# JoshElkind/concurrent-raytracer-go

Measured on AMD Instinct MI355X. Metric: Mrays/sec at 800x600x100spp max_depth=50 (sphere_reflections_light), higher is better.
Workload: dtype f64; 1 GPU; sphere_reflections_light_facing 800x600 100spp depth 50, soft shadows, recursive reflections; width=800, height=600, spp=100, max_depth=50, parallelism=1 GPU, frames_in_flight=64, frames_per_launch=32

## Files before the change

concurrent-raytracer-go_amd/csrc/rt_api.cpp:

```cpp
#include <math.h>
#include <stdlib.h>

#include <chrono>
#include <mutex>
#include <thread>

#include "rt_context.h"

namespace rtgo {

static thread_local std::string g_last_error;
void set_error(const std::string& msg) { g_last_error = msg; }

static int validate_scene(const rt_scene* s) {
  if (!s) {
    set_error("scene is NULL");
    return RT_E_INVALID;
  }
  if (s->num_objects < 0 || s->num_lights < 0 || (s->num_objects > 0 && !s->objects) ||
      (s->num_lights > 0 && !s->lights)) {
    set_error("scene arrays inconsistent");
    return RT_E_INVALID;
  }
  for (int i = 0; i < s->num_objects; ++i) {
// ... 221 lines not shown
  if (n > 0 && (!out || capacity < n)) {
    set_error("cone rows: out holds " + std::to_string(out ? capacity : 0) + " rows, the scene has " + std::to_string(n));
    return RT_E_INVALID;
  }
  FlatScene f;
  flatten_scene(*scene, &f);
  if ((force_bvh > 0 || (force_bvh == 0 && (f.spheres.size() > 64 || f.boxes.size() > (size_t)kAutoBvhCubes))) &&
      spheres_finite(f))
    build_bvh(&f, 0, 0);
  std::vector<unsigned long long> rows;
  cone_rows(f, &rows);
  for (size_t i = 0; i < n; ++i) out[i] = rows[i];
  return RT_OK;
}

int rt_stream_decode(int32_t order, uint32_t frames, uint32_t nlive, uint32_t spp, const uint32_t* entries, size_t n,
                     uint32_t* out) {
  if ((order != 0 && order != 1) || frames == 0 || nlive == 0 || spp == 0 || (n > 0 && (!entries || !out))) {
    set_error("stream decode: order is 0 or 1, frames, nlive and spp are at least 1, entries and out hold n");
    return RT_E_INVALID;
  }
  bool small = ((frames | nlive | spp) >> 31) == 0;
  for (size_t j = 0; j < n && small; ++j) small = (entries[j] >> 31) == 0;
  if (!small) {
    set_error("stream decode: frames, nlive, spp and every entry are below 2^31");
    return RT_E_INVALID;
  }
  const StreamDecode k = stream_decode_of(order, frames, nlive, spp);
  for (size_t j = 0; j < n; ++j) {
    const StreamEntry en = stream_decode(k, order, entries[j]);
    out[3 * j] = en.fl;
    out[3 * j + 1] = en.i;
    out[3 * j + 2] = en.s;
  }
  return RT_OK;
}

const char* rt_last_error(void) { return g_last_error.c_str(); }

constexpr size_t kStageDefault = 256 * 1024;
constexpr size_t kSmallDefault = 64 * 1024;

int rt_context_create(int32_t device, rt_context** out) {
  if (!out) {
    set_error("out is NULL");
    return RT_E_INVALID;
  }
  *out = nullptr;
  int n = 0;
  HIP_TRY(hipGetDeviceCount(&n));
  if (device < 0 || device >= n) {
    set_error("device " + std::to_string(device) + " out of range (" + std::to_string(n) + " devices)");
    return RT_E_DEVICE;
  }
  HIP_TRY(hipSetDevice(device));
  {
    static std::mutex mu;
    static std::vector<bool> loaded;
    std::lock_guard<std::mutex> lock(mu);
    if ((int)loaded.size() < n) loaded.resize(n, false);
    if (!loaded[device]) {
      hipError_t e = (hipError_t)preload_render_kernels();
      if (e == hipSuccess) e = (hipError_t)preload_sched_kernels();
      if (e == hipSuccess) e = (hipError_t)preload_wf_kernels();
      if (e != hipSuccess) {
        set_error(std::string("kernel code object load failed: ") + hipGetErrorString(e));
// ... 273 lines not shown
```

concurrent-raytracer-go_amd/csrc/rt_device.h:

```cpp
#pragma once
#include <hip/hip_runtime.h>

#include "../../include/rt_rng.h"
#include "rt_internal.h"

#ifdef RT_CHECK_XLANE
namespace rtgo {
__device__ unsigned long long g_xlane_faults;
}
template <typename T>
__device__ __forceinline__ T rt_checked_shfl(T v, int src, int width = 64) {
  const unsigned long long ex = __builtin_amdgcn_read_exec();
  const int lane = (int)(threadIdx.x & 63);
  const int from = (lane & ~(width - 1)) + (src & (width - 1));
  if (!((ex >> (from & 63)) & 1ull)) atomicAdd(&rtgo::g_xlane_faults, 1ull);
  return __shfl(v, src, width);
}
#define __shfl(...) rt_checked_shfl(__VA_ARGS__)
#endif

namespace rtgo {

struct d3 {
  double x, y, z;
// ... 112 lines not shown
__device__ __forceinline__ bool unit_ball_accept(uint32_t ux, uint32_t uy, uint32_t uz) {
  const float fx = __builtin_fmaf((float)ux, 0x1p-31f, -1.f), fy = __builtin_fmaf((float)uy, 0x1p-31f, -1.f),
              fz = __builtin_fmaf((float)uz, 0x1p-31f, -1.f);
  const float l = __builtin_fmaf(fz, fz, __builtin_fmaf(fy, fy, fx * fx));
  if (l < 1.f - 0x1p-16f) return true;
  if (l > 1.f + 0x1p-16f) return false;
  return len2(unit_ball_point(ux, uy, uz)) < 1;
}

template <bool kCount>
__device__ __forceinline__ d3 rand_in_unit_sphere(rt_rng& r, Counters& c) {
  for (;;) {
    const uint32_t ux = rt_rng_next(&r), uy = rt_rng_next(&r), uz = rt_rng_next(&r);
    cnt<kCount>(c, C_RNG, 3);
    if (unit_ball_accept(ux, uy, uz)) return unit_ball_point(ux, uy, uz);
  }
}

__device__ __forceinline__ double approx_rcp(double a) {
  const double r0 = __builtin_amdgcn_rcp(a);
  const double e = __builtin_fma(-a, r0, 1.0);
  return __builtin_fma(r0, e, r0);
}

__device__ __forceinline__ bool root_out(double num, double a, double inv_a, double tmin, double tmax) {
  const double r = num * inv_a;
  const double e = fabs(r) * 0x1p-40;
  if (r + e < tmin || r - e > tmax) return true;
  if (r - e >= tmin && r + e <= tmax) return false;
  const double q = num / a;
  return q < tmin || tmax < q;
}

__device__ __forceinline__ int sphere_query(const DSphere& S, d3 o, d3 d, double a, double inv_a, double tmin,
                                            double tmax, double& num) {
  double ocx = o.x - S.c[0], ocy = o.y - S.c[1], ocz = o.z - S.c[2];
  double hb = ocx * d.x + ocy * d.y + ocz * d.z;
  double c = (ocx * ocx + ocy * ocy + ocz * ocz) - S.r2;
  double disc = hb * hb - a * c;
  if (disc < 0) return 0;
  double sq = sqrt(disc);
  double n1 = -hb - sq;
  if (!root_out(n1, a, inv_a, tmin, tmax)) {
    num = n1;
    return 1;
  }
  double n2 = -hb + sq;
  if (!root_out(n2, a, inv_a, tmin, tmax)) {
    num = n2;
    return 2;
  }
  return 0;
}

__device__ __forceinline__ bool tri_test(const DTri& T, d3 o, d3 d, double tmin, double tmax, double& t,
                                         double& uo, double& vo) {
  d3 e1 = ld3(T.e1), e2 = ld3(T.e2);
  d3 h = cross(d, e2);
  double a = dot(e1, h);
  if (a > -1e-6 && a < 1e-6) return false;
  double f = 1.0 / a;
  d3 s = o - ld3(T.v0);
  double u = f * dot(s, h);
  if (u < 0.0 || u > 1.0) return false;
  d3 q = cross(s, e1);
  double v = f * dot(d, q);
  if (v < 0.0 || u + v > 1.0) return false;
  double tv = f * dot(e2, q);
  if (tv < tmin || tv > tmax) return false;
  t = tv;
  uo = u;
  vo = v;
  return true;
// ... 551 lines not shown
```

concurrent-raytracer-go_amd/csrc/rt_internal.h:

```cpp
#pragma once
#include <stdint.h>

#include <string>
#include <vector>

#include <hip/hip_runtime_api.h>

#include "../../include/rt_api.h"
#include "rt_scene_dev.h"

namespace rtgo {

void set_error(const std::string& msg);

int dev_alloc(void** p, size_t n);
void dev_free(void* p);
int host_alloc(void** p, size_t n, bool* fresh = nullptr);
void host_free(void* p);
int dev_stream_get(hipStream_t* s);
void dev_stream_put(hipStream_t s);
int dev_event_get(hipEvent_t* e);
void dev_event_put(hipEvent_t e);

struct FlatScene {
// ... 181 lines not shown
#define RT_HOST_DEVICE __host__ __device__
#else
#define RT_HOST_DEVICE
#endif
struct StreamDiv {
  uint32_t d, m, l, _pad;
};
struct StreamDecode {
  StreamDiv d0, d1;
};
struct StreamEntry {
  uint32_t fl, i, s;
};
inline StreamDiv stream_div_of(uint32_t d) {
  StreamDiv r{d, 0, 0, 0};
  while ((1ull << r.l) < d) ++r.l;
  r.m = (uint32_t)(((1ull << (31 + r.l)) + d - 1) / d);
  return r;
}
inline StreamDecode stream_decode_of(int32_t order, uint32_t frames, uint32_t nlive, uint32_t spp) {
  const uint32_t a = order == 0 ? spp : frames, b = order == 0 ? nlive : spp;
  return StreamDecode{stream_div_of(a ? a : 1u), stream_div_of(b ? b : 1u)};
}
template <class Div>
RT_HOST_DEVICE inline uint32_t stream_div(uint32_t n, const Div& k) {
  return (uint32_t)(((uint64_t)(n << 1) * k.m) >> 32) >> k.l;
}
template <class Decode>
RT_HOST_DEVICE inline StreamEntry stream_decode(const Decode& k, int32_t order, uint32_t e) {
  const uint32_t t = stream_div(e, k.d0), r0 = e - t * k.d0.d;
  const uint32_t q = stream_div(t, k.d1), r1 = t - q * k.d1.d;
  return order == 0 ? StreamEntry{q, r1, r0} : StreamEntry{r0, q, r1};
}
struct StreamParams {
  const int32_t* live;
  const int32_t* live_pos;
  const int32_t* tile_list;
  double* rows;
  unsigned int* cursor;
  uint32_t total;
  int32_t nlive, npix;
  int32_t frame0, frames;
  int32_t chunk, order;
  double* acc;
  const CamFrame* cams;
  StreamDecode dec;
};
struct StreamKArgs {
  KParams k;
  StreamParams s;
};
int launch_stream(const KParams& p, const StreamParams& sp, int wgs, void* stream);
constexpr int kStreamKernels = 6;
int stream_kernel_of(const KParams& p, bool cams = false);
struct CamTable {
  CamFrame f[kMaxFrames];
};
int launch_cam_upload(const CamTable& t, int n, CamFrame* d_cams, void* stream);
int stream_wave_slots(int device, int kernel, size_t shmem);

int launch_render(const KParams& p, bool count, void* stream);
size_t render_shmem(const KParams& p);
int launch_download(const void* d_src, void* h_dst_mapped, size_t bytes, void* stream);
int launch_spin(double ms, void* stream);
int partition_balanced(rt_context* c, int32_t w, int32_t h, const rt_settings* st, int32_t world, int measure_spp,
                       rt_partition** out);
// ... 146 lines not shown
```

concurrent-raytracer-go_amd/csrc/rt_kernel.hip:

```cpp
#include <hip/hip_runtime.h>

#include "../../include/rt_rng.h"
#include "rt_device.h"
#include "rt_internal.h"

#ifndef RT_WAVES_PER_SIMD
#define RT_WAVES_PER_SIMD 3
#endif
#ifndef RT_STREAM_SPH_WAVES
#define RT_STREAM_SPH_WAVES 4
#endif
#ifndef RT_COOP_MAX
#define RT_COOP_MAX 8
#endif
constexpr int kCoopMax = RT_COOP_MAX;
#ifndef RT_SQ_TAIL
#define RT_SQ_TAIL 2
#endif
constexpr int kSqTail = RT_SQ_TAIL;
#ifndef RT_SQ_TRIES
#define RT_SQ_TRIES 2
#endif
constexpr int kSqTries = RT_SQ_TRIES;
#ifndef RT_SOLO
// ... 63 lines not shown
      for (int j = 0; j < p.nb; ++j) {
        const DBox& B = p.boxes[j];
        const unsigned long long g = 0xFFFull << B.first;
        if ((m.t & g) && !ray_box(B, o, id, 0.001, tmax)) m.t &= ~g;
      }
    }
  }
  if (m.s) {
    const double a = len2(d);
    const double inv_a = approx_rcp(a);
    for (unsigned long long b = m.s; b; b &= b - 1) {
      const int i = __builtin_ctzll(b);
      cnt<kCount>(c, C_SPH);
      double num;
      if (sphere_query(p.spheres[i], o, d, a, inv_a, 0.001, tmax, num)) return true;
    }
  }
  if constexpr (!kSph) {
    for (unsigned long long b = m.t; b; b &= b - 1) {
      const int i = __builtin_ctzll(b);
      cnt<kCount>(c, C_TRI);
      double t, u, v;
      if (tri_test(p.tris[i], o, d, 0.001, tmax, t, u, v)) return true;
    }
  }
  return false;
}

template <bool kCount, bool kSph = false, bool kMix = false>
__device__ __forceinline__ bool shadow_blocked(const Geo& p, bool masks, d3 o, d3 d, double tmax,
                                               typename Kind<kSph>::C m, int* stack, Counters& c) {
  if (masks) return cand_any(m) && any_hit_masked<kCount, kSph>(p, o, d, tmax, m, c);
  return any_hit<kCount, kSph, kMix>(p, o, d, tmax, stack, c);
}

__device__ __forceinline__ int wide_groups(bool need, unsigned long long qmask, int nq, int* owner_tab, int& ow,
                                           int& k, bool& helper) {
  const int lane = (int)(threadIdx.x & 63);
  const int S = nq <= 4 ? 16 : (nq <= 8 ? 8 : 4);
  if (need) owner_tab[lanes_below(qmask)] = lane;
  __syncthreads();
  const int grp = lane / S;
  k = lane - grp * S;
  helper = grp < nq;
  ow = helper ? owner_tab[grp] : lane;
  __syncthreads();
  return S;
}

template <bool kCount, bool kSph = false>
__device__ __forceinline__ bool closest_wide(const Geo& g, bool need, unsigned long long qmask, int nq, d3 o, d3 d,
                                             typename Kind<kSph>::H& hs, bool& fallback, Counters& c) {
  __shared__ int owner_tab[16];
  const int lane = (int)(threadIdx.x & 63);
  int ow, k;
  bool helper;
  const int S = wide_groups(need, qmask, nq, owner_tab, ow, k, helper);
  const d3 ro = mk(__shfl(o.x, ow), __shfl(o.y, ow), __shfl(o.z, ow));
  const d3 rd = mk(__shfl(d.x, ow), __shfl(d.y, ow), __shfl(d.z, ow));
  const double a = len2(rd);
  const double inv_a = approx_rcp(a);
  double bt = __builtin_inf(), bnum = 0;
  int bobj = -1, bidx = -1;
  bool found = false;
  if (helper) {
    for (int i = k; i < g.ns; i += S) {
// ... 51 lines not shown
  unsigned long long m = 0;
  if (helper) {
    for (int i = k; i < g.ns; i += S) {
      const DSphere& Sp = g.spheres[i];
      if constexpr (kRows) {
        if (!((rowo >> i) & 1)) continue;
      }
      if (self_out && Sp.obj == selfo && Sp.r > 0) continue;
      if (in_cone(Sp.c, Sp.r, Po, Lo, dist)) m |= 1ull << i;
    }
  }
  for (int off = S >> 1; off >= 1; off >>= 1) m |= __shfl_xor(m, off);
  const int lead = need ? lanes_below(qmask) * S : lane;
  return __shfl(m, lead);
}

__device__ __forceinline__ bool light_inert(const DMat* m, const DLight& Lt, d3 N, d3 ldir, d3 D) {
  return gmax0(dot(N, ldir)) == 0.0 && D.x != 0.0 && D.y != 0.0 && D.z != 0.0 && __builtin_isfinite(Lt.intensity) &&
         __builtin_isfinite(Lt.color[0] + Lt.color[1] + Lt.color[2]) &&
         __builtin_isfinite(m->albedo[0] + m->albedo[1] + m->albedo[2]) && __builtin_isfinite(m->metallic) &&
         __builtin_isfinite(m->diffuse_strength);
}

struct CoopOut {
  uint64_t x;
  int unocc;
  int tries;
};
__device__ __forceinline__ Cand cand_of_lane(Cand m, int ow) { return Cand{rl64(m.s, ow), rl64(m.t, ow)}; }
__device__ __forceinline__ CandS cand_of_lane(CandS m, int ow) { return CandS{rl64(m.s, ow)}; }
template <bool kCount, bool kSph = false, bool kMix = false>
__device__ __forceinline__ CoopOut soft_coop(const Geo p, bool masks, bool trace, d3 P, d3 ldir, double ldist,
                             typename Kind<kSph>::C cm, uint64_t x, const uint64_t* jump, int* stack, Counters& c) {
  const int lane = (int)(threadIdx.x & 63);
  int need = 16, unocc = 0, tries = 0;
  while (need > 0) {
    const uint64_t x0 = state_at3(x, jump, lane), x1 = x0 * RT_PCG_MULT + RT_PCG_INC,
                   x2 = x1 * RT_PCG_MULT + RT_PCG_INC;
    const uint32_t o0 = rt_pcg_out(x0), o1 = rt_pcg_out(x1), o2 = rt_pcg_out(x2);
    const bool acc = unit_ball_accept(o0, o1, o2);
    const unsigned long long am = __ballot(acc);
    const int rank = lanes_below(am);
    const bool chosen = acc && rank < need;
    const unsigned long long chm = __ballot(chosen);
    const int nch = __popcll(chm);
    const int used = nch == need ? 64 - __clzll(chm) : 64;
    bool occ = false;
    if (chosen && trace)
      occ = shadow_blocked<kCount, kSph, kMix>(p, masks, P, normalize(ldir + muls(unit_ball_point(o0, o1, o2), 0.1)), ldist,
                                         cm, stack, c);
    unocc += nch - __popcll(__ballot(chosen && occ));
    need -= nch;
    tries += used;
    x = state_at3(x, jump, used);
  }
  return CoopOut{x, unocc, tries};
}

template <bool kCount, bool kSph = false, bool kMix = false>
__device__ __forceinline__ int soft_queue(const Geo& p, bool masks, bool need_soft, bool trace, d3 P, d3 ldir,
                                          double ldist, typename Kind<kSph>::C cm, rt_rng& rng, const uint64_t* jump,
                                          int* stack, Counters& c) {
  constexpr int kRingNeed = 64 * kSqTries + 64 + 16 * kSqTail;
  constexpr unsigned kRing = kRingNeed <= 256 ? 256u : (unsigned)kRingNeed;
  __shared__ uint4 sq[kRing];
  __shared__ int sq_unocc[64];
  const int lane = lane_now() & 63;
  sq_unocc[lane] = 0;
  int need = need_soft ? 16 : 0, free_rays = 0;
  int head = 0, tail = 0;
  for (;;) {
    constexpr int K = kSqTries;
    bool acc[K];
    uint32_t u[K][3];
#pragma unroll
    for (int t = 0; t < K; ++t) {
      acc[t] = false;
      u[t][0] = u[t][1] = u[t][2] = 0;
    }
    if (need > 0) {
      rt_rng r = rng;
#pragma unroll
      for (int t = 0; t < K; ++t) {
// ... 38 lines not shown
            const int nch = __popcll(chm);
            const int used = nch == nd ? 64 - __clzll(chm) : 64;
            if (tr) {
              if (chosen) sq[(unsigned)(tail + lanes_below(chm)) % kRing] = make_uint4(o0, o1, o2, (uint32_t)ow);
              tail += nch;
            }
            got += nch;
            nd -= nch;
            tries += used;
            x = state_at3(x, jump, used);
          }
          if (lane == ow) {
            rng.x = x;
            need = 0;
            if (!tr) free_rays += got;
            cnt<kCount>(c, C_RNG, 3ull * tries);
            cnt<kCount>(c, C_SHADOW, got);
          }
        }
      }
    }
    const bool more = __ballot(need > 0) != 0;
    while (tail - head >= 64 || (!more && tail > head)) {
      __syncthreads();
      const int n = min(64, tail - head);
      const uint4 e = sq[(unsigned)(head + lane) % kRing];
      const int ow = lane < n ? (int)e.w : lane;
      const d3 Po = mk(__shfl(P.x, ow), __shfl(P.y, ow), __shfl(P.z, ow));
      const d3 Lo = mk(__shfl(ldir.x, ow), __shfl(ldir.y, ow), __shfl(ldir.z, ow));
      const double dist = __shfl(ldist, ow);
      typename Kind<kSph>::C co;
      co.s = __shfl(cm.s, ow);
      if constexpr (!kSph) co.t = p.nt ? __shfl(cm.t, ow) : 0ull;
      if (lane < n) {
        const d3 pt = mk(rt_bits_to_unit(e.x) * 2 - 1, rt_bits_to_unit(e.y) * 2 - 1, rt_bits_to_unit(e.z) * 2 - 1);
        if (!shadow_blocked<kCount, kSph, kMix>(p, masks, Po, normalize(Lo + muls(pt, 0.1)), dist, co, stack, c))
          atomicAdd(&sq_unocc[ow], 1);
      }
      head += n;
      __syncthreads();
    }
    if (!more && head == tail) break;
  }
  __syncthreads();
  return need_soft ? sq_unocc[lane] + free_rays : 0;
}


typedef const __attribute__((address_space(4))) KParams* KArg;
__device__ __forceinline__ KArg fresh() {
  KArg k = (KArg)__builtin_amdgcn_kernarg_segment_ptr();
  asm volatile("" : "+s"(k));
  return k;
}

__device__ __forceinline__ unsigned main_wg(KArg k) {
  const unsigned b = blockIdx.x;
  return (k->tail != nullptr && b >= (unsigned)k->tail_pos) ? b - (unsigned)k->tail_helpers : b;
}
__device__ __forceinline__ int frame_of(KArg k) {
  return k->nframes > 1 ? (int)(main_wg(k) % (unsigned)k->nframes) : 0;
}
__device__ __forceinline__ int block_of(KArg k) {
  return k->nframes > 1 ? (int)(main_wg(k) / (unsigned)k->nframes) : (int)main_wg(k);
}
__device__ __forceinline__ size_t split_index(KArg k, int slot) {
  return (size_t)frame_of(k) * (size_t)k->nsplit + (size_t)slot;
}

struct BlockLoc {
  int lt, tile, tx, ty;
// ... 84 lines not shown
    const bool mine = ((row >> i) & 1) != 0 && !(sphere_out && S.obj == self && S.r > 0);
    if (__ballot(mine) == 0) continue;
    if (mine && in_cone(S.c, S.r, P, ldir, ldist)) m.s |= 1ull << i;
  }
  return m;
}

__device__ __forceinline__ CamK cam_k(KArg k) {
  return make_cam(k->frame_key[frame_of(k)], k->W, k->H, k->cf);
}
template <bool kCount>
__device__ __forceinline__ void camera_ray(KArg k, int x, int y, int s, rt_rng& rng, d3& o, d3& d, Counters& c) {
  camera_ray_c<kCount>(cam_k(k), k->cf, x, y, s, rng, o, d, c);
}

enum WgSection { kClkHit, kClkLight, kClkSoft, kClkHard, kClkScat };
#ifdef RT_WG_TIMING
__shared__ unsigned long long solo_clk[16];
struct WgClock {
  unsigned long long t_start = 0, t_loop = 0, iter = 0;
  unsigned long long sec[5] = {0, 0, 0, 0, 0}, from[5] = {0, 0, 0, 0, 0};
  unsigned long long vis = 0, alive = 0, coop = 0, seq = 0;
  unsigned long long rf_top = 0, rf_top_lanes = 0, rf_second = 0, rf_second_lanes = 0;
  typedef unsigned long long Buckets __attribute__((ext_vector_type(5)));
  Buckets bclk = {0, 0, 0, 0, 0}, bcnt = {0, 0, 0, 0, 0};
  unsigned long long bts = 0;
  int bprev = -1;
  unsigned long long solo_t0 = 0;
  unsigned long long first = 0, last = 0, last_d0 = 0, last_d1 = 0, paths = 0, solo = 0, bounces = 0;

  __device__ __forceinline__ unsigned long long* record(KArg k) const { return k->dbg + (size_t)blockIdx.x * kDbgStride; }
  __device__ __forceinline__ void start(int lane) {
    if (lane < 16) solo_clk[lane] = 0;
    t_start = __builtin_amdgcn_s_memrealtime();
    vis = __builtin_amdgcn_s_memtime();
  }
  __device__ __forceinline__ void visibility_done() { vis = __builtin_amdgcn_s_memtime() - vis; }
  __device__ __forceinline__ void iteration(bool is_alive, int lane) {
    ++iter;
    alive += __popcll(__ballot(is_alive));
    {
      const unsigned long long now = __builtin_amdgcn_s_memtime();
      if (bprev >= 0) bclk[bprev] += now - bts;
      const int nal = __popcll(__ballot(is_alive));
      bprev = nal == 1 ? 0 : (nal == 2 ? 1 : (nal <= 4 ? 2 : (nal <= 8 ? 3 : 4)));
      bcnt[bprev] += 1;
      bts = now;
    }
    if (iter % 4 == 0 && iter / 4 < 16 && lane == 0 && fresh()->dbg) record(fresh())[16 + iter / 4] = __builtin_amdgcn_s_memrealtime();
    from[kClkHit] = __builtin_amdgcn_s_memtime();
  }
  __device__ __forceinline__ void begin(WgSection s) { from[s] = __builtin_amdgcn_s_memtime(); }
  __device__ __forceinline__ void end(WgSection s) { sec[s] += __builtin_amdgcn_s_memtime() - from[s]; }
  __device__ __forceinline__ void hit_done() {
    from[kClkLight] = __builtin_amdgcn_s_memtime();
    sec[kClkHit] += from[kClkLight] - from[kClkHit];
  }
  __device__ __forceinline__ void soft_form(unsigned long long owners) {
    if (__popcll(owners) <= kCoopMax) coop += __popcll(owners); else ++seq;
  }
  __device__ __forceinline__ void refill(bool second, unsigned long long served) {
    if (served == 0) return;
    if (second) {
      rf_second += 1;
      rf_second_lanes += __popcll(served);
    } else {
      rf_top += 1;
      rf_top_lanes += __popcll(served);
    }
  }
  __device__ __forceinline__ void loop_done() {
    t_loop = __builtin_amdgcn_s_memrealtime();
    if (bprev >= 0) bclk[bprev] += __builtin_amdgcn_s_memtime() - bts;
  }
  __device__ __forceinline__ void write(KArg k, int lane, bool block, unsigned long long shape, unsigned long long split) const {
    if (k->dbg && lane == 0) {
      unsigned long long* r = record(k);
      r[0] = t_start;
      r[1] = t_loop;
      r[2] = __builtin_amdgcn_s_memrealtime();
      r[3] = sec[kClkHit];
      r[4] = sec[kClkLight];
      r[5] = sec[kClkSoft];
      r[6] = vis;
      r[7] = iter;
      r[8] = sec[kClkHard];
      r[9] = sec[kClkScat];
      r[10] = alive;
      r[11] = coop;
      r[12] = seq;
      r[13] = shape;
      r[14] = split;
      for (int i = 0; i < 5; ++i) {
        r[32 + i] = bclk[i];
        r[37 + i] = bcnt[i];
      }
      if (block && solo_clk[6])
        for (int i = 0; i < 16; ++i) r[16 + i] = solo_clk[i];
      r[42] = block ? solo_clk[6] : 0;
      r[43] = block ? solo_clk[7] : 0;
      r[44] = rf_top;
      r[45] = rf_top_lanes;
      r[46] = rf_second;
      r[47] = rf_second_lanes;
    }
  }
  __device__ __forceinline__ void stream_write(int lane) const { write(fresh(), lane, false, 0, 0); }
  __device__ __forceinline__ void solo_start() { solo_t0 = __builtin_amdgcn_s_memtime(); }
  __device__ __forceinline__ void solo_count(int k) { solo_clk[k] += 1; }
  __device__ __forceinline__ void solo_lap(int k) {
    const unsigned long long now = __builtin_amdgcn_s_memtime();
    solo_clk[k] += now - solo_t0;
    solo_t0 = now;
  }
  __device__ __forceinline__ void solo_mark(int k) { solo_clk[k] += __builtin_amdgcn_s_memtime() - solo_t0; }
  __device__ __forceinline__ void helper_path(unsigned long long t_path, int d0, int d1) {
    if (!first) first = t_path;
    paths += 1;
    solo += __builtin_amdgcn_s_memrealtime() - t_path;
    last = t_path;
    last_d0 = (unsigned long long)d0;
    last_d1 = (unsigned long long)d1;
    bounces += (unsigned long long)(d1 - d0);
  }
  __device__ __forceinline__ void helper_write(KArg k, int lane, unsigned long long t_born) const {
// ... 1951 lines not shown
```

concurrent-raytracer-go_amd/rtgo/__init__.py:

```python
from __future__ import annotations

import ctypes
import json
import os
import time
from datetime import datetime, timezone

import numpy as np

_HERE = os.path.dirname(os.path.abspath(__file__))
LIB_PATH = os.environ.get("RTGO_LIB") or os.path.join(os.path.dirname(_HERE), "build", "librtgo.so")

RT_OK = 0
RT_E_TIMEOUT = -6
RT_OBJ_SPHERE, RT_OBJ_CUBE = 0, 1
MATERIAL_KINDS = {
    "lambertian": 0,
    "metal": 1,
    "shiny": 2,
    "perfectmirror": 3,
    "glass": 4,
    "dielectric": 5,
    "diffuselight": 6,
}
# ... 235 lines not shown
    "rt_partition_tile",
    "rt_partition_max_local",
    "rt_partition_packed_bytes",
    "rt_partition_rgba_offset",
    "rt_partition_work",
    "rt_context_set_partition",
    "rt_unpack_partition_async",
    "rt_comm_gather_bytes_async",
    "rt_renderer_rank_seconds",
    "rt_renderer_num_ranks",
    "rt_debug_xlane_faults",
    "rt_context_tail_debug",
    "rt_context_profile",
    "rt_context_kernel_seconds",
    "rt_context_render_frames_async",
    "rt_unpack_partition_frames_async",
    "rt_release_cached_memory",
    "rt_renderer_set_watchdog",
    "rt_renderer_test_stall",
    "rt_context_get_stats",
    "rt_context_progressive_begin",
    "rt_context_progressive_add_async",
    "rt_context_progressive_samples",
    "rt_context_progressive_end",
    "rt_rgba_delta_async",
    "rt_context_progressive_set_adaptive",
    "rt_context_progressive_counts_async",
    "rt_context_progressive_state",
    "rt_adaptive_step",
    "rt_scene_cone_rows",
    "rt_context_render_cameras_async",
    "rt_camera_orbit",
    "rt_stream_decode",
]

_lib = None


def lib():
    global _lib
    if _lib is not None:
        return _lib
    if not os.path.exists(LIB_PATH):
        raise RenderError(
            f"{LIB_PATH} is missing: build it with `make -C concurrent-raytracer-go_amd` "
            "(or __graft_entry__.build())"
        )
    if os.environ.get("RTGO_NO_TORCH", "0") != "1":
        try:
            import torch
        except ImportError:
            pass
    L = ctypes.CDLL(LIB_PATH)
    vp, i32, sz = ctypes.c_void_p, ctypes.c_int32, ctypes.c_size_t
    sig = {
        "rt_settings_default": (None, [ctypes.POINTER(Settings)]),
        "rt_abi_version": (i32, []),
        "rt_last_error": (ctypes.c_char_p, []),
        "rt_scene_load_json": (ctypes.c_int, [ctypes.c_char_p, i32, ctypes.POINTER(vp)]),
        "rt_scene_parse_json": (ctypes.c_int, [ctypes.c_char_p, sz, i32, ctypes.POINTER(vp)]),
        "rt_scene_view": (ctypes.POINTER(SceneView), [vp]),
        "rt_scene_warnings": (i32, [vp]),
        "rt_scene_free": (None, [vp]),
        "rt_scene_print_hittables": (ctypes.c_int, [vp]),
        "rt_render": (
            ctypes.c_int,
# ... 52 lines not shown
        "rt_context_profile": (ctypes.c_int, [vp, i32]),
        "rt_context_render_frames_async": (
            ctypes.c_int,
            [vp, i32, i32, ctypes.POINTER(Settings), i32, ctypes.POINTER(ctypes.c_uint64), i32, i32, i32,
             ctypes.POINTER(vp), ctypes.POINTER(vp), vp],
        ),
        "rt_unpack_partition_frames_async": (ctypes.c_int, [vp, i32, vp, vp, vp, vp]),
        "rt_release_cached_memory": (ctypes.c_int, []),
        "rt_renderer_set_watchdog": (ctypes.c_int, [vp, ctypes.c_double]),
        "rt_renderer_test_stall": (ctypes.c_int, [vp, i32, ctypes.c_double]),
        "rt_context_get_stats": (ctypes.c_int, [vp, ctypes.POINTER(ContextStats)]),
        "rt_context_kernel_seconds": (ctypes.c_int, [vp, ctypes.POINTER(ctypes.c_double),
                                                     ctypes.POINTER(ctypes.c_int64)]),
        "rt_context_progressive_begin": (ctypes.c_int, [vp, i32, i32, ctypes.POINTER(Settings), i32, i32, i32]),
        "rt_context_progressive_add_async": (ctypes.c_int, [vp, i32, vp, vp, vp]),
        "rt_context_progressive_samples": (ctypes.c_int64, [vp]),
        "rt_context_progressive_end": (ctypes.c_int, [vp]),
        "rt_rgba_delta_async": (ctypes.c_int, [vp, vp, sz, vp, vp]),
        "rt_context_progressive_set_adaptive": (ctypes.c_int, [vp, ctypes.POINTER(Adaptive)]),
        "rt_context_progressive_counts_async": (ctypes.c_int, [vp, vp, vp]),
        "rt_context_progressive_state": (ctypes.c_int, [vp, ctypes.POINTER(ctypes.c_int64)]),
        "rt_adaptive_step": (ctypes.c_int, [ctypes.POINTER(ctypes.c_uint8), ctypes.POINTER(ctypes.c_uint8), i32, i32,
                                             i32, ctypes.POINTER(Adaptive), ctypes.POINTER(i32)]),
        "rt_camera_frame": (ctypes.c_int, [ctypes.POINTER(Camera), i32, i32, i32, ctypes.POINTER(ctypes.c_double)]),
        "rt_scene_cone_rows": (ctypes.c_int, [ctypes.POINTER(SceneView), i32, ctypes.POINTER(ctypes.c_uint64), sz]),
        "rt_context_render_cameras_async": (
            ctypes.c_int,
            [vp, i32, i32, ctypes.POINTER(Settings), i32, ctypes.POINTER(Camera), ctypes.POINTER(ctypes.c_uint64), i32,
             i32, i32, ctypes.POINTER(vp), ctypes.POINTER(vp), vp],
        ),
        "rt_camera_orbit": (ctypes.c_int, [ctypes.POINTER(Camera), i32, ctypes.c_double, ctypes.POINTER(Camera)]),
        "rt_stream_decode": (ctypes.c_int, [i32, ctypes.c_uint32, ctypes.c_uint32, ctypes.c_uint32,
                                             ctypes.POINTER(ctypes.c_uint32), sz, ctypes.POINTER(ctypes.c_uint32)]),
    }
    for name, (res, args) in sig.items():
        f = getattr(L, name)
        f.restype = res
        f.argtypes = args
    _lib = L
    return L


def _check(rc):
    if rc != RT_OK:
        msg = lib().rt_last_error()
        raise RenderError(f"librtgo error {rc}: {msg.decode() if msg else ''}")


def default_settings() -> Settings:
    s = Settings()
    lib().rt_settings_default(ctypes.byref(s))
    return s


def default_tuning(**over) -> Tuning:
    t = Tuning()
    lib().rt_tuning_default(ctypes.byref(t))
    for k, v in over.items():
        setattr(t, k, v)
    return t


class Scene:

    def __init__(self, handle=None, objects=None, lights=None, camera=None):
        self._handle = handle
# ... 521 lines not shown

def camera_orbit(camera, n: int, degrees: float = 360.0) -> list:
    n = int(n)
    cam = _as_camera(camera)
    out = (Camera * max(1, n))()
    _check(lib().rt_camera_orbit(ctypes.byref(cam), n, float(degrees), out))
    return [_camera_dict(out[k]) for k in range(n)]


def camera_frame(camera, model, width: int, height: int) -> np.ndarray:
    camera = _as_camera(camera)
    out = np.zeros(12, np.float64)
    _check(lib().rt_camera_frame(ctypes.byref(camera), CAMERAS.get(model, model), width, height,
                                 out.ctypes.data_as(ctypes.POINTER(ctypes.c_double))))
    return out


def cone_rows(scene: Scene, force_bvh: int = 0) -> np.ndarray:
    nl, no = int(scene.view.num_lights), int(scene.view.num_objects)
    out = np.zeros(max(nl * no, 1), np.uint64)
    _check(lib().rt_scene_cone_rows(ctypes.byref(scene.view), force_bvh,
                                    out.ctypes.data_as(ctypes.POINTER(ctypes.c_uint64)), out.size))
    return out[: nl * no].reshape(nl, no)


def stream_decode(order: int, frames: int, nlive: int, spp: int, entries) -> np.ndarray:
    e = np.ascontiguousarray(entries, np.uint32)
    out = np.zeros((max(e.size, 1), 3), np.uint32)
    u32p = ctypes.POINTER(ctypes.c_uint32)
    _check(lib().rt_stream_decode(order, frames, nlive, spp, e.ctypes.data_as(u32p), e.size, out.ctypes.data_as(u32p)))
    return out[: e.size]


def render(scene: Scene, width: int, height: int, settings: Settings):
    lin = np.zeros((height, width, 3), np.float32)
    rgba = np.zeros((height, width, 4), np.uint8)
    st = Stats()
    _check(lib().rt_render(ctypes.byref(scene.view), width, height, ctypes.byref(settings), lin.ctypes.data,
                           rgba.ctypes.data, ctypes.byref(st)))
    return rgba, lin, st


def adaptive_step(old_rgba, new_rgba, had_image, count: int, streak: int, tolerance: int, patience: int = 1,
                  min_samples: int = 0):
    o = (ctypes.c_uint8 * 4)(*[int(v) for v in old_rgba])
    n = (ctypes.c_uint8 * 4)(*[int(v) for v in new_rgba])
    a = Adaptive(int(tolerance), int(patience), int(min_samples), 0)
    ns = ctypes.c_int32(0)
    rc = lib().rt_adaptive_step(o, n, 1 if had_image else 0, int(count), int(streak), ctypes.byref(a), ctypes.byref(ns))
    if rc < 0:
        _check(rc)
    return bool(rc), int(ns.value)


def rgba_delta_async(d_a: int, d_b: int, npix: int, d_out: int, stream: int = 0):
    _check(lib().rt_rgba_delta_async(ctypes.c_void_p(d_a), ctypes.c_void_p(d_b), npix, ctypes.c_void_p(d_out),
                                     ctypes.c_void_p(stream)))


def max_local_tiles(width: int, height: int, world: int) -> int:
    return lib().rt_max_local_tiles(width, height, world)


def packed_bytes(width: int, height: int, world: int) -> int:
    return lib().rt_packed_bytes(width, height, world)

# ... 111 lines not shown
```

include/rt_api.h:

```cpp
#ifndef RT_API_H
#define RT_API_H

#include <stddef.h>
#include <stdint.h>

#ifdef __cplusplus
extern "C" {
#endif

#define RT_ABI_VERSION 8

#define RT_OK 0
#define RT_E_INVALID (-1)
#define RT_E_IO (-2)
#define RT_E_PARSE (-3)
#define RT_E_DEVICE (-4)
#define RT_E_NOMEM (-5)
#define RT_E_TIMEOUT (-6)

#define RT_OBJ_SPHERE 0
#define RT_OBJ_CUBE 1

#define RT_MAT_LAMBERTIAN 0
#define RT_MAT_METAL 1
// ... 97 lines not shown
  uint64_t culled[9];
  uint64_t soft_occlusion[9];
  uint64_t extend[9];
  uint64_t hard_occlusion[9];
} rt_counts;

void rt_settings_default(rt_settings* s);
int rt_release_cached_memory(void);
int32_t rt_abi_version(void);
int rt_debug_xlane_faults(int32_t device, int32_t reset, uint64_t* out);
const char* rt_last_error(void);


typedef struct rt_scene_buf rt_scene_buf;

int rt_scene_load_json(const char* path, int32_t verbose, rt_scene_buf** out);
int rt_scene_parse_json(const char* text, size_t len, int32_t verbose, rt_scene_buf** out);
const rt_scene* rt_scene_view(const rt_scene_buf* buf);
int32_t rt_scene_warnings(const rt_scene_buf* buf);
void rt_scene_free(rt_scene_buf* buf);
int rt_scene_print_hittables(const rt_scene_buf* buf);


int rt_render(const rt_scene* scene, int32_t width, int32_t height, const rt_settings* settings,
              float* out_linear_rgb, uint8_t* out_rgba, rt_stats* stats);
int rt_validate(const rt_scene* scene, int32_t width, int32_t height, const rt_settings* settings);

int rt_camera_frame(const rt_camera* cam, int32_t model, int32_t width, int32_t height, double out[12]);

int rt_scene_cone_rows(const rt_scene* scene, int32_t force_bvh, uint64_t* out, size_t capacity);

int rt_stream_decode(int32_t order, uint32_t frames, uint32_t nlive, uint32_t spp, const uint32_t* entries, size_t n,
                     uint32_t* out);


typedef struct rt_renderer rt_renderer;
int rt_renderer_create(const int32_t* devices, int32_t num_devices, rt_renderer** out);
int rt_renderer_render(rt_renderer* r, const rt_scene* scene, int32_t width, int32_t height,
                       const rt_settings* settings, float* out_linear_rgb, uint8_t* out_rgba, rt_stats* stats);
void rt_renderer_destroy(rt_renderer* r);
int rt_renderer_set_watchdog(rt_renderer* r, double seconds);
int rt_renderer_test_stall(rt_renderer* r, int32_t rank, double ms);


typedef struct rt_context rt_context;

int rt_context_create(int32_t device, rt_context** out);
void rt_context_destroy(rt_context* ctx);

int rt_context_set_scene(rt_context* ctx, const rt_scene* scene, int32_t force_bvh);

#define RT_PATH_AUTO 0
#define RT_PATH_MEGAKERNEL 1
typedef struct {
  int32_t path;
  int32_t pilot;
  int32_t frustum;
  int32_t stage;
  double block_work;
  int32_t block_samples;
  int32_t bvh_bins;
  int32_t bvh_leaf;
  int32_t wf_paths;
  int64_t wf_chunk;
  int32_t wf_lds_nodes;
  int32_t wf_trav_block;
// ... 139 lines not shown
```

Baseline: 460,100 Mrays/s.

## Add conservative sphere shadow pre-screen using unnormalized direction and fast rsqrt

Adds a soft_screen test that decides hit or miss for sphere shadow rays from an unnormalized jittered direction with a float rsqrt estimate of its inverse length, scaling the quadratic terms and comparing against error margins. Only undecided cases fall back to the exact normalize-and-test shadow path. It targets the sqrt, normalize and divide cost in soft shadow sampling for sphere scenes. In exchange it adds extra arithmetic per candidate sphere, may duplicate work when results are undecided, and adds debug timing hooks plus a host test API.

```diff
diff --git a/concurrent-raytracer-go_amd/csrc/rt_api.cpp b/concurrent-raytracer-go_amd/csrc/rt_api.cpp
--- a/concurrent-raytracer-go_amd/csrc/rt_api.cpp
+++ b/concurrent-raytracer-go_amd/csrc/rt_api.cpp
@@ -277,6 +277,20 @@
     out[3 * j] = en.fl;
     out[3 * j + 1] = en.i;
     out[3 * j + 2] = en.s;
+  }
+  return RT_OK;
+}
+
+static_assert(kSoftUndecided == RT_SOFT_UNDECIDED && kSoftMiss == RT_SOFT_MISS && kSoftHit == RT_SOFT_HIT, "rt_api.h");
+int rt_soft_screen(const double* centers, const double* r2, const double* origins, const double* dirs, const double* il,
+                   const double* tmin, const double* tmax, size_t n, int32_t* out) {
+  if (n > 0 && (!centers || !r2 || !origins || !dirs || !il || !tmin || !tmax || !out)) {
+    set_error("soft screen: every array holds n cases");
+    return RT_E_INVALID;
+  }
+  for (size_t j = 0; j < n; ++j) {
+    const double *c = centers + 3 * j, *o = origins + 3 * j, *u = dirs + 3 * j;
+    out[j] = soft_screen(c[0], c[1], c[2], r2[j], o[0], o[1], o[2], u[0], u[1], u[2], il[j], tmin[j], tmax[j]);
   }
   return RT_OK;
 }
diff --git a/concurrent-raytracer-go_amd/csrc/rt_device.h b/concurrent-raytracer-go_amd/csrc/rt_device.h
--- a/concurrent-raytracer-go_amd/csrc/rt_device.h
+++ b/concurrent-raytracer-go_amd/csrc/rt_device.h
@@ -168,6 +168,17 @@
   return q < tmin || tmax < q;
 }
 
+#ifndef RT_SOFT_SCREEN
+#define RT_SOFT_SCREEN 1
+#endif
+#ifdef RT_WG_TIMING
+__shared__ unsigned int soft_note_flag;
+__shared__ unsigned long long soft_pass_cnt[2];
+__device__ __forceinline__ void soft_note() { soft_note_flag = 1; }
+#else
+__device__ __forceinline__ void soft_note() {}
+#endif
+
 __device__ __forceinline__ int sphere_query(const DSphere& S, d3 o, d3 d, double a, double inv_a, double tmin,
                                             double tmax, double& num) {
   double ocx = o.x - S.c[0], ocy = o.y - S.c[1], ocz = o.z - S.c[2];
@@ -175,6 +186,7 @@
   double c = (ocx * ocx + ocy * ocy + ocz * ocz) - S.r2;
   double disc = hb * hb - a * c;
   if (disc < 0) return 0;
+  if (!RT_SOFT_SCREEN) soft_note();
   double sq = sqrt(disc);
   double n1 = -hb - sq;
   if (!root_out(n1, a, inv_a, tmin, tmax)) {
diff --git a/concurrent-raytracer-go_amd/csrc/rt_internal.h b/concurrent-raytracer-go_amd/csrc/rt_internal.h
--- a/concurrent-raytracer-go_amd/csrc/rt_internal.h
+++ b/concurrent-raytracer-go_amd/csrc/rt_internal.h
@@ -237,6 +237,38 @@
   const uint32_t q = stream_div(t, k.d1), r1 = t - q * k.d1.d;
   return order == 0 ? StreamEntry{q, r1, r0} : StreamEntry{r0, q, r1};
 }
+constexpr int kSoftScreenBits = 17;
+constexpr int kSoftScreenBits2 = 16;
+constexpr double kSoftScreenIl = 2e-7;
+enum SoftScreen { kSoftUndecided = 0, kSoftMiss = 1, kSoftHit = 2 };
+RT_HOST_DEVICE inline double soft_scaled(double x) { return __builtin_ldexp(x, kSoftScreenBits); }
+RT_HOST_DEVICE inline int soft_screen(double cx, double cy, double cz, double r2, double px, double py, double pz,
+                                      double ux, double uy, double uz, double il, double tmin, double tmax) {
+  if (!(tmin >= 0x1p-40 && tmin <= tmax && tmax < 0x1p500)) return kSoftUndecided;
+  const double ocx = px - cx, ocy = py - cy, ocz = pz - cz;
+  const double o2 = __builtin_fma(ocz, ocz, __builtin_fma(ocy, ocy, ocx * ocx));
+  const double h = __builtin_fma(ocz, uz, __builtin_fma(ocy, uy, ocx * ux)) * il;
+  const double cc = o2 - r2, q = o2 + __builtin_fabs(r2);
+  if (!(q < 0x1p1000)) return kSoftUndecided;
+  const double q2 = __builtin_ldexp(q, -kSoftScreenBits2);
+  const double D = soft_scaled(__builtin_fma(h, h, -cc)), mD = __builtin_fma(h, h, q2);
+  if (-D > mD) return kSoftMiss;
+  const double ah = __builtin_fabs(h);
+  const double g0 = soft_scaled(__builtin_fma(tmin, __builtin_fma(2.0, h, tmin), cc));
+  const double m0 = __builtin_fma(tmin, __builtin_fma(2.0, ah, tmin), q2);
+  const double g1 = soft_scaled(__builtin_fma(tmax, __builtin_fma(2.0, h, tmax), cc));
+  const double m1 = __builtin_fma(tmax, __builtin_fma(2.0, ah, tmax), q2);
+  const bool p0 = g0 > m0, n0 = -g0 > m0, p1 = g1 > m1, n1 = -g1 > m1;
+  if ((p0 && n1) || (n0 && p1)) return kSoftHit;
+  if (n0 && n1) return kSoftMiss;
+  if (p0 && p1) {
+    const double v0 = soft_scaled(tmin + h), v1 = soft_scaled(tmax + h), w0 = tmin + ah, w1 = tmax + ah;
+    if (v0 > w0 || -v1 > w1) return kSoftMiss;
+    if (-v0 > w0 && v1 > w1 && D > mD) return kSoftHit;
+  }
+  return kSoftUndecided;
+}
+
 struct StreamParams {
   const int32_t* live;
   const int32_t* live_pos;
diff --git a/concurrent-raytracer-go_amd/csrc/rt_kernel.hip b/concurrent-raytracer-go_amd/csrc/rt_kernel.hip
--- a/concurrent-raytracer-go_amd/csrc/rt_kernel.hip
+++ b/concurrent-raytracer-go_amd/csrc/rt_kernel.hip
@@ -119,6 +119,39 @@
                                                typename Kind<kSph>::C m, int* stack, Counters& c) {
   if (masks) return cand_any(m) && any_hit_masked<kCount, kSph>(p, o, d, tmax, m, c);
   return any_hit<kCount, kSph, kMix>(p, o, d, tmax, stack, c);
+}
+
+template <bool kCount, bool kMix>
+__device__ __forceinline__ bool soft_blocked_sph(const Geo& p, bool masks, d3 P, d3 ldir, d3 pt, double ldist, CandS m,
+                                                 int* stack, Counters& c) {
+  if (RT_SOFT_SCREEN && masks) {
+    const d3 u = ldir + muls(pt, 0.1);
+    const double il = (double)__builtin_amdgcn_rsqf((float)__builtin_fma(u.z, u.z, __builtin_fma(u.y, u.y, u.x * u.x)));
+    bool undecided = false;
+    for (unsigned long long b = m.s; b; b &= b - 1) {
+      const DSphere& S = p.spheres[__builtin_ctzll(b)];
+      const int r = soft_screen(S.c[0], S.c[1], S.c[2], S.r2, P.x, P.y, P.z, u.x, u.y, u.z, il, 0.001, ldist);
+      if (r == kSoftHit) return true;
+      undecided |= r == kSoftUndecided;
+    }
+    if (!undecided) return false;
+    soft_note();
+  }
+  return shadow_blocked<kCount, true, kMix>(p, masks, P, normalize(ldir + muls(pt, 0.1)), ldist, m, stack, c);
+}
+__device__ __forceinline__ void soft_pass_begin(int lane) {
+#ifdef RT_WG_TIMING
+  if (lane == 0) soft_note_flag = 0;
+#endif
+}
+__device__ __forceinline__ void soft_pass_done(int lane) {
+#ifdef RT_WG_TIMING
+  if (lane == 0) {
+    soft_pass_cnt[0] += 1;
+    soft_pass_cnt[1] += soft_note_flag;
+    soft_note_flag = 0;
+  }
+#endif
 }
 
 __device__ __forceinline__ int wide_groups(bool need, unsigned long long qmask, int nq, int* owner_tab, int& ow,
@@ -236,7 +269,7 @@
 template <bool kCount, bool kSph = false, bool kMix = false>
 __device__ __forceinline__ CoopOut soft_coop(const Geo p, bool masks, bool trace, d3 P, d3 ldir, double ldist,
                              typename Kind<kSph>::C cm, uint64_t x, const uint64_t* jump, int* stack, Counters& c) {
-  const int lane = (int)(threadIdx.x & 63);
+  const int lane = kSph ? lane_now() & 63 : (int)(threadIdx.x & 63);
   int need = 16, unocc = 0, tries = 0;
   while (need > 0) {
     const uint64_t x0 = state_at3(x, jump, lane), x1 = x0 * RT_PCG_MULT + RT_PCG_INC,
@@ -250,9 +283,15 @@
     const int nch = __popcll(chm);
     const int used = nch == need ? 64 - __clzll(chm) : 64;
     bool occ = false;
-    if (chosen && trace)
-      occ = shadow_blocked<kCount, kSph, kMix>(p, masks, P, normalize(ldir + muls(unit_ball_point(o0, o1, o2), 0.1)), ldist,
-                                         cm, stack, c);
+    if constexpr (kSph) {
+      if (trace) soft_pass_begin(lane);
+      if (chosen && trace) occ = soft_blocked_sph<kCount, kMix>(p, masks, P, ldir, unit_ball_point(o0, o1, o2), ldist, cm, stack, c);
+      if (trace) soft_pass_done(lane);
+    } else {
+      if (chosen && trace)
+        occ = shadow_blocked<kCount, kSph, kMix>(p, masks, P, normalize(ldir + muls(unit_ball_point(o0, o1, o2), 0.1)), ldist,
+                                           cm, stack, c);
+    }
     unocc += nch - __popcll(__ballot(chosen && occ));
     need -= nch;
     tries += used;
@@ -357,11 +396,17 @@
       typename Kind<kSph>::C co;
       co.s = __shfl(cm.s, ow);
       if constexpr (!kSph) co.t = p.nt ? __shfl(cm.t, ow) : 0ull;
+      if constexpr (kSph) soft_pass_begin(lane);
       if (lane < n) {
         const d3 pt = mk(rt_bits_to_unit(e.x) * 2 - 1, rt_bits_to_unit(e.y) * 2 - 1, rt_bits_to_unit(e.z) * 2 - 1);
-        if (!shadow_blocked<kCount, kSph, kMix>(p, masks, Po, normalize(Lo + muls(pt, 0.1)), dist, co, stack, c))
-          atomicAdd(&sq_unocc[ow], 1);
-      }
+        bool blocked;
+        if constexpr (kSph)
+          blocked = soft_blocked_sph<kCount, kMix>(p, masks, Po, Lo, pt, dist, co, stack, c);
+        else
+          blocked = shadow_blocked<kCount, kSph, kMix>(p, masks, Po, normalize(Lo + muls(pt, 0.1)), dist, co, stack, c);
+        if (!blocked) atomicAdd(&sq_unocc[ow], 1);
+      }
+      if constexpr (kSph) soft_pass_done(lane);
       head += n;
       __syncthreads();
     }
@@ -512,6 +557,7 @@
   __device__ __forceinline__ unsigned long long* record(KArg k) const { return k->dbg + (size_t)blockIdx.x * kDbgStride; }
   __device__ __forceinline__ void start(int lane) {
     if (lane < 16) solo_clk[lane] = 0;
+    if (lane < 2) soft_pass_cnt[lane] = 0;
     t_start = __builtin_amdgcn_s_memrealtime();
     vis = __builtin_amdgcn_s_memtime();
   }
@@ -571,6 +617,7 @@
       r[12] = seq;
       r[13] = shape;
       r[14] = split;
+      r[15] = soft_pass_cnt[0] | soft_pass_cnt[1] << 32;
       for (int i = 0; i < 5; ++i) {
         r[32 + i] = bclk[i];
         r[37 + i] = bcnt[i];
diff --git a/concurrent-raytracer-go_amd/rtgo/__init__.py b/concurrent-raytracer-go_amd/rtgo/__init__.py
--- a/concurrent-raytracer-go_amd/rtgo/__init__.py
+++ b/concurrent-raytracer-go_amd/rtgo/__init__.py
@@ -291,6 +291,7 @@
     "rt_context_render_cameras_async",
     "rt_camera_orbit",
     "rt_stream_decode",
+    "rt_soft_screen",
 ]
 
 _lib = None
@@ -409,6 +410,7 @@
         "rt_camera_orbit": (ctypes.c_int, [ctypes.POINTER(Camera), i32, ctypes.c_double, ctypes.POINTER(Camera)]),
         "rt_stream_decode": (ctypes.c_int, [i32, ctypes.c_uint32, ctypes.c_uint32, ctypes.c_uint32,
                                              ctypes.POINTER(ctypes.c_uint32), sz, ctypes.POINTER(ctypes.c_uint32)]),
+        "rt_soft_screen": (ctypes.c_int, [ctypes.POINTER(ctypes.c_double)] * 7 + [sz, ctypes.POINTER(i32)]),
     }
     for name, (res, args) in sig.items():
         f = getattr(L, name)
@@ -996,6 +998,22 @@
     return out[: e.size]
 
 
+SOFT_UNDECIDED, SOFT_MISS, SOFT_HIT = 0, 1, 2
+
+
+def soft_screen(centers, r2, origins, dirs, il, tmin, tmax) -> np.ndarray:
+    c, o, u = (np.ascontiguousarray(a, np.float64).reshape(-1, 3) for a in (centers, origins, dirs))
+    n = c.shape[0]
+    assert o.shape[0] == n and u.shape[0] == n, (c.shape, o.shape, u.shape)
+    s = [np.ascontiguousarray(np.broadcast_to(np.asarray(a, np.float64), (n,))) for a in (r2, il, tmin, tmax)]
+    out = np.zeros(max(n, 1), np.int32)
+    dp = ctypes.POINTER(ctypes.c_double)
+    _check(lib().rt_soft_screen(c.ctypes.data_as(dp), s[0].ctypes.data_as(dp), o.ctypes.data_as(dp), u.ctypes.data_as(dp),
+                                s[1].ctypes.data_as(dp), s[2].ctypes.data_as(dp), s[3].ctypes.data_as(dp), n,
+                                out.ctypes.data_as(ctypes.POINTER(ctypes.c_int32))))
+    return out[:n]
+
+
 def render(scene: Scene, width: int, height: int, settings: Settings):
     lin = np.zeros((height, width, 3), np.float32)
     rgba = np.zeros((height, width, 4), np.uint8)
diff --git a/include/rt_api.h b/include/rt_api.h
--- a/include/rt_api.h
+++ b/include/rt_api.h
@@ -153,6 +153,12 @@
 
 int rt_stream_decode(int32_t order, uint32_t frames, uint32_t nlive, uint32_t spp, const uint32_t* entries, size_t n,
                      uint32_t* out);
+
+#define RT_SOFT_UNDECIDED 0
+#define RT_SOFT_MISS 1
+#define RT_SOFT_HIT 2
+int rt_soft_screen(const double* centers, const double* r2, const double* origins, const double* dirs, const double* il,
+                   const double* tmin, const double* tmax, size_t n, int32_t* out);
 
 
 typedef struct rt_renderer rt_renderer;
```

Measured after the change: 475,000 Mrays/s (median of 6 runs). +3.3%, better.
